# leejaeyong7/nerfacc

Hardware: AMD Instinct MI355X
Metric: rays/sec (fwd+bwd) through 128^3 occ-grid, 1M-ray batch (higher is better)
Workload: dtype f32; 1 GPU; cfg2: 1048576 image rays/GPU, 128^3 shell10 occ grid (G=1), step 2*sqrt(3)/1024, sampling+rendering fwd+bwd; rays_per_gpu=1048576, resolution=128, grid=shell10, samples_after_compaction=32244949, parallelism=ray-sharded x1, field=synthetic analytic field, native callbacks (see bench.py NativeField/TorchField)

## Files before the change

### include/nerfacc_hip.h

```cpp
#ifndef NERFACC_HIP_H
#define NERFACC_HIP_H

#include <stdint.h>

#ifdef __cplusplus
extern "C" {
#endif

#define NFA_OK 0
#define NFA_EINVAL (-1)
#define NFA_EHIP (-2)

#define NFA_MAX_GRID_LEVELS 8

typedef void *nfa_stream_t;

#define NFA_ELEM_F32 0
#define NFA_ELEM_F16 1
#define NFA_ELEM_BF16 2

const char *nfa_last_error(void);
#define NFA_VERSION 403
int nfa_version(void);
int nfa_set_tuning(const char *name, const char *value);
int nfa_device_arch(char *buf, int buflen);


int64_t nfa_cumsum_scratch_bytes(int64_t n);
int nfa_exclusive_cumsum_i64(const int64_t *cnts, int64_t n, int64_t *starts, int64_t *total,
                             void *scratch, nfa_stream_t stream);
int nfa_exclusive_cumsum_pairs_i64(const int64_t *cnts, int64_t n, int64_t *packed_info , int64_t *total,
                                   void *scratch, nfa_stream_t stream);
int nfa_exclusive_cumsum_pairs_stats_i64(const int64_t *cnts, int64_t n, int64_t *packed_info ,
                                         int64_t *total_and_stats , void *scratch, nfa_stream_t stream);

int nfa_pack_info(const int64_t *ray_indices, int64_t n, int64_t n_rays, int64_t *packed_info ,
                  int32_t *flags , void *scratch, nfa_stream_t stream);

int nfa_unpack_rows(const void *packed, const int64_t *packed_info , const uint8_t *mask, int64_t n_rays,
                    int64_t n_per_ray, int64_t n_packed, int64_t row_bytes, const void *pad_host, int32_t pad_bytes,
                    void *padded, nfa_stream_t stream);
int nfa_pack_rows(const void *padded, const int64_t *packed_info , const uint8_t *mask, int64_t n_rays,
                  int64_t n_per_ray, int64_t n_packed, int64_t row_bytes, void *packed, nfa_stream_t stream);
int nfa_mask_row_counts(const uint8_t *mask, int64_t n_rows, int64_t n_cols, int64_t *counts, nfa_stream_t stream);

int nfa_pack_bits(const uint8_t *binaries, int64_t n_cells, uint32_t *bits , nfa_stream_t stream);


int nfa_ray_aabb_intersect(const float *rays_o, const float *rays_d, int64_t n_rays,
// ... 384 lines not shown
```

### nerfacc_amd/_backend.py

```python
from __future__ import annotations

import ctypes as C
import os
import threading
from typing import Optional

import torch

from . import _build

_lock = threading.Lock()
_lib: Optional[C.CDLL] = None

_vp, _i64, _i32, _f32, _u64, _int = C.c_void_p, C.c_int64, C.c_int32, C.c_float, C.c_uint64, C.c_int


class TraverseArgs(C.Structure):
    _fields_ = [
        ("n_rays", _i64), ("rays_o", _vp), ("rays_d", _vp), ("rays_mask", _vp),
        ("n_grids", _i32), ("res", _i32 * 3), ("binaries", _vp), ("aabbs", _vp),
        ("hits", _vp), ("t_sorted", _vp), ("t_indices", _vp),
        ("near_planes", _vp), ("far_planes", _vp),
        ("step_size", _f32), ("cone_angle", _f32), ("traverse_steps_limit", _i32), ("mode", _i32),
        ("iv_vals", _vp), ("iv_ray_indices", _vp), ("iv_is_left", _vp), ("iv_is_right", _vp),
        ("iv_starts", _vp), ("iv_cnts", _vp),
        ("sm_vals", _vp), ("sm_ray_indices", _vp), ("sm_is_valid", _vp),
        ("sm_t_starts", _vp), ("sm_t_ends", _vp), ("sm_starts", _vp), ("sm_cnts", _vp),
        ("terminate_planes", _vp),
        ("ray_filter", _vp), ("ray_filter_min", _i32),
        ("bricks", _vp), ("coarse", _vp),
        ("steps_limit_dev", _vp), ("n_listed_dev", _vp), ("run_if_nonzero", _vp),
    ]


_SIGS = {
    "nfa_exclusive_cumsum_i64": [_vp, _i64, _vp, _vp, _vp, _vp],
    "nfa_exclusive_cumsum_pairs_i64": [_vp, _i64, _vp, _vp, _vp, _vp],
    "nfa_exclusive_cumsum_pairs_stats_i64": [_vp, _i64, _vp, _vp, _vp, _vp],
    "nfa_pack_info": [_vp, _i64, _i64, _vp, _vp, _vp, _vp],
    "nfa_pdf_loss_fwd": [_vp, _vp, _vp, _vp, _i64, _i32, _i32, _f32, _vp, _vp, _vp],
    "nfa_pdf_loss_bwd": [_vp, _vp, _vp, _i64, _i32, _i32, _f32, _vp, _vp, _vp, _vp],
    "nfa_pdf_loss_partials": [_i64, _i32, _i32],
    "nfa_pdf_loss_sum_fwd": [_vp, _vp, _vp, _vp, _i64, _i32, _i32, _f32, _vp, _vp, _vp],
    "nfa_pdf_loss_mean_bwd": [_vp, _vp, _vp, _i64, _i32, _i32, _f32, _vp, _vp, _vp, _vp],
    "nfa_pack_bits": [_vp, _i64, _vp, _vp],
    "nfa_unpack_rows": [_vp, _vp, _vp, _i64, _i64, _i64, _i64, _vp, _i32, _vp, _vp],
    "nfa_pack_rows": [_vp, _vp, _vp, _i64, _i64, _i64, _i64, _vp, _vp],
    "nfa_mask_row_counts": [_vp, _i64, _i64, _vp, _vp],
    "nfa_ray_aabb_intersect": [_vp, _vp, _i64, _vp, _i32, _f32, _f32, _f32, _vp, _vp, _vp, _vp],
    "nfa_ray_events": [_vp, _vp, _i64, _vp, _i32, _vp, _vp, _vp, _vp],
    "nfa_traverse_grids": [C.POINTER(TraverseArgs), _vp],
    "nfa_bricks_words": [_i32, C.POINTER(_i32)],
    "nfa_pack_bricks": [_vp, _i32, C.POINTER(_i32), _vp, _vp, _vp],
# ... 176 lines not shown
            dev = t.device
        elif t.device != dev:
            raise RuntimeError(f"nerfacc_amd: tensors on different devices ({dev} vs {t.device})")
    if dev is None:
        raise RuntimeError("nerfacc_amd: no tensor argument")
    return dev


def seg_plan(n_elems: int, n_rays: int = 0):
    t, n = _i64(0), _i64(0)
    load().nfa_seg_plan(n_elems, n_rays, C.byref(t), C.byref(n))
    return int(t.value), int(n.value)


def cumsum_scratch(n: int, device) -> torch.Tensor:
    nbytes = ((max(n, 1) + 2047) // 2048 + 1) * 8
    return torch.empty(nbytes // 8, dtype=torch.int64, device=device)
```

### nerfacc_amd/_segments.py

```python
from __future__ import annotations

import ctypes
import weakref
from dataclasses import dataclass
from typing import Optional

import torch
from torch import Tensor

from . import _backend as B


@dataclass
class SegInfo:
    packed_info: Tensor
    n_rays: int
    n_elems: int
    tiles: Optional[Tensor]
    contiguous: bool
    sorted_indices: bool = True
    n_tiles: int = 0
    trusted: bool = False


_ATTR = "_nfa_seg"
_ATTR_RI = "_nfa_seg_from_ray_indices"


def _build_tiles(packed_info: Tensor, n_elems: int, trusted: bool) -> SegInfo:
    dev = B.require_device(packed_info)
    n_rays = packed_info.shape[0]
    with torch.cuda.device(dev):
        tile_elems, n_tiles = B.seg_plan(n_elems, n_rays)
        tiles = torch.empty((int(B.load().nfa_seg_table_rows(n_tiles)), 2), dtype=torch.int64, device=dev)
        flag = None if trusted else torch.empty(1, dtype=torch.int32, device=dev)
        B.call("nfa_seg_build_tiles", B.ptr(packed_info), n_rays, n_elems, tile_elems, n_tiles, B.ptr(tiles), B.ptr(flag),
               B.stream())
        ok = True if trusted else (int(flag.item()) == 0)
    return SegInfo(packed_info, n_rays, n_elems, tiles if ok else None, ok, n_tiles=n_tiles, trusted=trusted)


def seginfo_from_packed(packed_info: Tensor, n_elems: int, trusted: bool = False) -> SegInfo:
    assert packed_info.dim() == 2 and packed_info.shape[-1] == 2, "packed_info must be 2-D with shape (B, 2)."
    cached = getattr(packed_info, _ATTR, None)
    if cached is not None and cached[0] == packed_info._version and cached[1] == n_elems:
        return cached[2]
    pi = packed_info
    if pi.dtype != torch.int64 or not pi.is_contiguous():
        pi = pi.to(torch.int64).contiguous()
    info = _build_tiles(pi, n_elems, trusted)
    try:
        setattr(packed_info, _ATTR, (packed_info._version, n_elems, info))
    except Exception:
        pass
    return info


def tag_trusted(packed_info: Tensor, n_elems: int) -> SegInfo:
    return seginfo_from_packed(packed_info, n_elems, trusted=True)


def pack_info_native(ray_indices: Tensor, n_rays: int):
    dev = B.require_device(ray_indices)
    ri = ray_indices if (ray_indices.dtype == torch.int64 and ray_indices.is_contiguous()) else \
        ray_indices.to(torch.int64).contiguous()
    with torch.cuda.device(dev):
        packed = torch.empty((n_rays, 2), dtype=torch.int64, device=dev)
        flag = torch.empty(1, dtype=torch.int32, device=dev)
        scratch = B.cumsum_scratch(n_rays, dev)
        B.call("nfa_pack_info", B.ptr(ri), ri.numel(), n_rays, B.ptr(packed), B.ptr(flag), B.ptr(scratch), B.stream())
    return packed, flag


def seginfo_from_ray_indices(ray_indices: Tensor, n_rays: int) -> SegInfo:
# ... 90 lines not shown
```

### nerfacc_amd/csrc/common.hip.h

```cpp
#pragma once
#include <hip/hip_runtime.h>
#include <stdint.h>
#include <stdio.h>
#include <stdlib.h>
#include <string.h>

#include <type_traits>

#include "../../include/nerfacc_hip.h"

#define NFA_WAVE 64

namespace nfa {

void set_error(const char *fmt, ...);

#define NFA_REQUIRE(cond, ...)                         \
    do {                                               \
        if (!(cond)) {                                 \
            nfa::set_error(__VA_ARGS__);               \
            return NFA_EINVAL;                         \
        }                                              \
    } while (0)

// ... 22 lines not shown
    int min_busy = 48;
    if (refill_env) { long c = 0; int m = 0; if (sscanf(refill_env, "%ld,%d", &c, &m) == 2 && c >= 64 && m >= 1 && m <= 64) { chunk = c / 64 * 64; min_busy = m; } }
    return RefillPlan{true, chunk, min_busy};
}

static inline hipStream_t as_stream(nfa_stream_t s) { return reinterpret_cast<hipStream_t>(s); }

__host__ __device__ static inline int64_t ceil_div64(int64_t a, int64_t b) { return (a + b - 1) / b; }

static inline unsigned grid_1d(int64_t n, int block, int64_t cap = 256 * 16)
{
    int64_t g = ceil_div64(n, block);
    if (g > cap) g = cap;
    if (g < 1) g = 1;
    return (unsigned)g;
}

static inline bool aligned16(const void *p) { return (reinterpret_cast<uintptr_t>(p) & 15) == 0; }
template <typename... P>
static inline bool all_aligned16(P... p) { return (aligned16(p) && ...); }

template <class F>
static void dispatch_bool(bool b, F &&f)
{
    if (b) f(std::true_type{});
    else f(std::false_type{});
}
template <class F>
static void dispatch_channels(int c, F &&f)
{
// ... 322 lines not shown
```

### nerfacc_amd/csrc/grid.hip

```cpp
#include <stdarg.h>

#include "common.hip.h"
#include "march.h"

namespace nfa {

static thread_local char g_err[512] = "";
void set_error(const char *fmt, ...)
{
    va_list ap;
    va_start(ap, fmt);
    vsnprintf(g_err, sizeof(g_err), fmt, ap);
    va_end(ap);
}

struct TuningKnob { char name[32]; char value[64]; };
static TuningKnob g_knobs[8];
static int g_n_knobs = 0;
const char *tuning_env(const char *name)
{
    for (int i = 0; i < g_n_knobs; ++i)
        if (strcmp(g_knobs[i].name, name) == 0) return g_knobs[i].value[0] ? g_knobs[i].value : nullptr;
    return nullptr;
}
// ... 340 lines not shown
        if (!span_cell<EMIT_RUNS, false, true, true>(a, tid, 0, 0, sp, st, ro)) return RF_WALK;
        return (a.traverse_steps_limit > 0 && st.n_samples >= a.traverse_steps_limit) ? RF_FINISH : RF_SPAN;
    }
    __device__ __forceinline__ void finish() { run_ray_close(a, ro, tid, st.t_last, st.n_samples, st.n_runs); }
};
template <bool FUSED>
__global__ __launch_bounds__(256) void traverse_refill_kernel(const nfa_traverse_args a, const RunOut ro, const int32_t chunk,
                                                              const int32_t min_busy)
{
    SpanState sp;
    BrickWalker<FUSED> w{a, ro, 0, 0, 0.0f, 0.0f, {0.0f, 0.0f, 0.0f}, {0.0f, 0.0f, 0.0f}, {0.0f, 0.0f, 0.0f}, RayState{0.0f, 0, 0, 0, -1, 0u, 0u, 0, 0}, sp};
    refill_schedule(w, ro.order, ro.order ? ro.n_order : a.n_rays, (int64_t)blockIdx.x * (blockDim.x >> 6) + (threadIdx.x >> 6), chunk, min_busy);
}

constexpr int CS_THREADS = 256;
constexpr int CS_ITEMS = 8;
constexpr int CS_BLOCK = CS_THREADS * CS_ITEMS;

__device__ __forceinline__ int64_t block_excl_scan_i64(int64_t v, int64_t &block_total, int64_t *lds )
{
    const int lane = lane_id(), wave = threadIdx.x >> 6;
    const int64_t incl = wave_incl_sum_i64(v);
    if (lane == 63) lds[wave] = incl;
    __syncthreads();
    int64_t wave_off = 0, tot = 0;
#pragma unroll
    for (int w = 0; w < CS_THREADS / 64; ++w) {
        const int64_t x = lds[w];
        if (w < wave) wave_off += x;
        tot += x;
    }
    __syncthreads();
    block_total = tot;
    return wave_off + incl - v;
}

__global__ __launch_bounds__(CS_THREADS) void cumsum_partials_kernel(const int64_t *__restrict__ in, int64_t n,
                                                                      int64_t in_stride, int64_t *__restrict__ partials)
{
    __shared__ int64_t lds[8];
    const int64_t base = (int64_t)blockIdx.x * CS_BLOCK + (int64_t)threadIdx.x * CS_ITEMS;
    int64_t s = 0;
#pragma unroll
    for (int k = 0; k < CS_ITEMS; ++k)
        if (base + k < n) s += in[(base + k) * in_stride];
    int64_t tot;
    block_excl_scan_i64(s, tot, lds);
    if (threadIdx.x == 0) partials[blockIdx.x] = tot;
}

__global__ __launch_bounds__(CS_THREADS) void cumsum_spine_kernel(int64_t *partials, int64_t n_blocks, int64_t *total)
{
    __shared__ int64_t lds[8];
    int64_t carry = 0;
    for (int64_t base = 0; base < n_blocks; base += CS_THREADS) {
        const int64_t i = base + threadIdx.x;
        const int64_t v = i < n_blocks ? partials[i] : 0;
        int64_t tot;
        const int64_t ex = block_excl_scan_i64(v, tot, lds);
        if (i < n_blocks) partials[i] = carry + ex;
        carry += tot;
    }
    if (threadIdx.x == 0 && total) *total = carry;
}

template <bool SPINE>
__global__ __launch_bounds__(CS_THREADS) void cumsum_final_kernel(const int64_t *__restrict__ in, int64_t n,
                                                                   int64_t in_stride,
                                                                   const int64_t *__restrict__ partials,
                                                                   int64_t *__restrict__ out, int pairs,
                                                                   int64_t *__restrict__ total,
                                                                   unsigned long long *__restrict__ stats = nullptr)
{
    __shared__ int64_t lds[8];
    int64_t block_off = 0;
    if (SPINE) {
        int64_t before = 0;
        for (int64_t j = threadIdx.x; j < (int64_t)blockIdx.x; j += CS_THREADS) before += partials[j];
        block_excl_scan_i64(before, block_off, lds);
    } else {
        block_off = partials[blockIdx.x];
    }
    const int64_t base = (int64_t)blockIdx.x * CS_BLOCK + (int64_t)threadIdx.x * CS_ITEMS;
    int64_t v[CS_ITEMS];
    int64_t s = 0;
#pragma unroll
    for (int k = 0; k < CS_ITEMS; ++k) {
        v[k] = (base + k < n) ? in[(base + k) * in_stride] : 0;
        s += v[k];
    }
    int64_t tot;
    int64_t run = block_off + block_excl_scan_i64(s, tot, lds);
    if (SPINE && total && blockIdx.x == gridDim.x - 1 && threadIdx.x == 0) *total = block_off + tot;
    if (SPINE && stats && (blockIdx.x & 7) == 0) {
        int64_t m = 0;
#pragma unroll
        for (int k = 0; k < CS_ITEMS; ++k) m = v[k] > m ? v[k] : m;
        for (int off = 1; off < 8; off <<= 1) { const int64_t u = __shfl_xor(m, off, 64); m = u > m ? u : m; }
        int64_t gm = (lane_id() & 7) == 0 ? m : 0;
        for (int off = 8; off < 64; off <<= 1) gm += __shfl_xor(gm, off, 64);
        if (lane_id() == 0) atomicAdd(&stats[0], (unsigned long long)gm);
        if (threadIdx.x == 0) atomicAdd(&stats[1], (unsigned long long)tot);
    }
#pragma unroll
    for (int k = 0; k < CS_ITEMS; ++k) {
        if (base + k < n) {
            if (pairs) { out[2 * (base + k)] = run; out[2 * (base + k) + 1] = v[k]; }
            else out[base + k] = run;
        }
        run += v[k];
    }
}

static int run_cumsum(const int64_t *in, int64_t n, int64_t in_stride, int64_t *out, int pairs, int64_t *total,
                      void *scratch, hipStream_t s, unsigned long long *stats = nullptr)
{
    const int64_t n_blocks = ceil_div64(n > 0 ? n : 1, CS_BLOCK);
    int64_t *partials = reinterpret_cast<int64_t *>(scratch);
    hipLaunchKernelGGL(cumsum_partials_kernel, dim3((unsigned)n_blocks), dim3(CS_THREADS), 0, s, in, n, in_stride, partials);
    if (n_blocks <= 2048) {
        hipLaunchKernelGGL(cumsum_final_kernel<true>, dim3((unsigned)n_blocks), dim3(CS_THREADS), 0, s, in, n, in_stride, partials,
                           out, pairs, total, stats);
    } else {
        hipLaunchKernelGGL(cumsum_spine_kernel, dim3(1), dim3(CS_THREADS), 0, s, partials, n_blocks, total);
        hipLaunchKernelGGL(cumsum_final_kernel<false>, dim3((unsigned)n_blocks), dim3(CS_THREADS), 0, s, in, n, in_stride, partials,
                           out, pairs, nullptr, nullptr);
    }
    NFA_CHECK_LAUNCH("exclusive_cumsum_i64");
    return NFA_OK;
}

__global__ __launch_bounds__(256) void pack_hist_kernel(const int64_t *__restrict__ ray_indices, int64_t n,
                                                        int64_t n_rays, unsigned long long *__restrict__ packed,
                                                        int32_t *__restrict__ flags)
{
    const int lane = lane_id();
    for (int64_t base = ((int64_t)blockIdx.x * blockDim.x + threadIdx.x) - lane; base < n;
         base += (int64_t)blockDim.x * gridDim.x) {
        const int64_t i = base + lane;
        const bool valid = i < n;
        const int64_t r = valid ? ray_indices[i] : -1;
        int64_t prev = __shfl_up(r, 1, NFA_WAVE);
// ... 57 lines not shown
    hipDeviceProp_t prop;
    if (hipGetDevice(&dev) != hipSuccess || hipGetDeviceProperties(&prop, dev) != hipSuccess) {
        set_error("no HIP device");
        return NFA_EHIP;
    }
    snprintf(buf, buflen, "%s", prop.gcnArchName);
    return NFA_OK;
}

int64_t nfa_cumsum_scratch_bytes(int64_t n) { return (ceil_div64(n > 0 ? n : 1, CS_BLOCK) + 1) * 8; }

int nfa_exclusive_cumsum_i64(const int64_t *cnts, int64_t n, int64_t *starts, int64_t *total, void *scratch,
                             nfa_stream_t stream)
{
    NFA_REQUIRE(n >= 0 && scratch && (n == 0 || (cnts && starts)), "exclusive_cumsum_i64: bad arguments");
    return run_cumsum(cnts, n, 1, starts, 0, total, scratch, as_stream(stream));
}

int nfa_exclusive_cumsum_pairs_i64(const int64_t *cnts, int64_t n, int64_t *packed_info, int64_t *total, void *scratch,
                                   nfa_stream_t stream)
{
    NFA_REQUIRE(n >= 0 && scratch && (n == 0 || (cnts && packed_info)), "exclusive_cumsum_pairs_i64: bad arguments");
    return run_cumsum(cnts, n, 1, packed_info, 1, total, scratch, as_stream(stream));
}

int nfa_exclusive_cumsum_pairs_stats_i64(const int64_t *cnts, int64_t n, int64_t *packed_info, int64_t *total_and_stats,
                                         void *scratch, nfa_stream_t stream)
{
    NFA_REQUIRE(n >= 0 && scratch && total_and_stats && (n == 0 || (cnts && packed_info)),
                "exclusive_cumsum_pairs_stats_i64: bad arguments");
    return run_cumsum(cnts, n, 1, packed_info, 1, total_and_stats, scratch, as_stream(stream),
                      reinterpret_cast<unsigned long long *>(total_and_stats + 1));
}

int nfa_pack_info(const int64_t *ray_indices, int64_t n, int64_t n_rays, int64_t *packed_info, int32_t *flags,
                  void *scratch, nfa_stream_t stream)
{
    NFA_REQUIRE(n >= 0 && n_rays >= 0 && flags && scratch, "pack_info: bad arguments");
    NFA_REQUIRE(n_rays == 0 || packed_info, "pack_info: packed_info is null");
    NFA_REQUIRE(n == 0 || ray_indices, "pack_info: ray_indices is null");
    hipStream_t s = as_stream(stream);
    hipLaunchKernelGGL(zero_i64_kernel, dim3(grid_1d(2 * n_rays + 1, 256)), dim3(256), 0, s, packed_info, 2 * n_rays, flags);
    if (n > 0 && n_rays > 0)
        hipLaunchKernelGGL(pack_hist_kernel, dim3(grid_1d(n, 256)), dim3(256), 0, s, ray_indices, n, n_rays,
                           reinterpret_cast<unsigned long long *>(packed_info), flags);
    NFA_CHECK_LAUNCH("pack_info");
    if (n_rays == 0) return NFA_OK;
    return run_cumsum(packed_info + 1, n_rays, 2, packed_info, 1, nullptr, scratch, s);
}

int nfa_pack_bits(const uint8_t *binaries, int64_t n_cells, uint32_t *bits, nfa_stream_t stream)
{
    NFA_REQUIRE(n_cells >= 0 && (n_cells == 0 || (binaries && bits)), "pack_bits: bad arguments");
    if (n_cells == 0) return NFA_OK;
    hipLaunchKernelGGL(pack_bits_kernel, dim3(grid_1d(n_cells, 256)), dim3(256), 0, as_stream(stream), binaries, n_cells, bits);
    NFA_CHECK_LAUNCH("pack_bits");
    return NFA_OK;
}

int nfa_ray_aabb_intersect(const float *rays_o, const float *rays_d, int64_t n_rays, const float *aabbs,
                           int32_t n_aabbs, float near_plane, float far_plane, float miss_value, float *t_mins,
                           float *t_maxs, uint8_t *hits, nfa_stream_t stream)
{
// ... 113 lines not shown
```

### nerfacc_amd/csrc/segscan.hip

```cpp
#include <stdlib.h>

#include "common.hip.h"
#include "samples.h"

namespace nfa {

constexpr int SE = 4;
constexpr int SQ = SE / 4;
constexpr int SEG_CHUNK = 64 * SE;
#ifndef NFA_SEG_TILE_ROWS
#define NFA_SEG_TILE_ROWS 256
#endif
constexpr int64_t SEG_TILE_ROWS = NFA_SEG_TILE_ROWS;
#ifndef NFA_VIS_EXP_FREE
#define NFA_VIS_EXP_FREE 1
#endif
#ifndef NFA_SEG_WAVES_PER_BLOCK
#define NFA_SEG_WAVES_PER_BLOCK 4
#endif
constexpr int SEG_WAVES_PER_BLOCK = NFA_SEG_WAVES_PER_BLOCK;

__global__ __launch_bounds__(256) void seg_build_tiles_kernel(const int64_t *__restrict__ packed_info, int64_t n_rays,
                                                              int64_t n_elems, int64_t tile_elems, int64_t n_tiles,
                                                              longlong2 *__restrict__ tiles, int32_t *__restrict__ flags)
{
    for (int64_t r = (int64_t)blockIdx.x * blockDim.x + threadIdx.x; r <= n_rays;
         r += (int64_t)blockDim.x * gridDim.x) {
        int64_t b_lo, b_hi, e_first;
        bool bad = false;
        if (r < n_rays) {
            const int64_t s = packed_info[2 * r], n = packed_info[2 * r + 1];
            int64_t s_prev = -1;
            if (r > 0) {
                const int64_t ps = packed_info[2 * r - 2], pn = packed_info[2 * r - 1];
                s_prev = ps;
                bad |= (ps + pn != s);
            }
            bad |= (n < 0) || (s < 0) || (s + n > n_elems);
            if (bad) { if (flags) atomicOr(flags, 1); continue; }
            b_lo = (s_prev < 0) ? 0 : s_prev / tile_elems + (r - 1) / SEG_TILE_ROWS + 1;
            b_hi = s / tile_elems + r / SEG_TILE_ROWS;
            e_first = s;
        } else {
            const int64_t s_prev = n_rays > 0 ? packed_info[2 * n_rays - 2] : -1;
            const int64_t n_prev = n_rays > 0 ? packed_info[2 * n_rays - 1] : 0;
            b_lo = (s_prev < 0) ? 0 : s_prev / tile_elems + (n_rays - 1) / SEG_TILE_ROWS + 1;
            b_hi = n_tiles;
            e_first = (s_prev < 0) ? 0 : s_prev + n_prev;
            if (s_prev > n_elems) { if (flags) atomicOr(flags, 1); continue; }
        }
        for (int64_t b = b_lo; b <= b_hi && b <= n_tiles; ++b) tiles[b] = make_longlong2(r, e_first);
    }
}

__host__ __device__ inline int64_t seg_table_rows(int64_t n_tiles) { return n_tiles + 1; }

struct F4 { float v[SE]; };

struct Pos {
    int64_t c;
    int32_t off;
// ... 2094 lines not shown
            op.gsig = grad_sigmas; op.grgb = grad_rgbs;
            launch_seg<-1>(op, packed_info, tiles, n_rays, n_tiles, as_stream(stream));
        });
    });
    NFA_CHECK_LAUNCH(name);
    return NFA_OK;
}

extern "C" {

void nfa_seg_plan(int64_t n_elems, int64_t n_rays, int64_t *tile_elems, int64_t *n_tiles)
{
    const int64_t t_env = tuning_env("NFA_SEG_TILE") ? atoll(tuning_env("NFA_SEG_TILE")) : 0;
    const int64_t t = t_env > 0 ? t_env : 1024;
    *tile_elems = t;
    *n_tiles = n_elems / t + (n_rays > 0 ? n_rays : 0) / SEG_TILE_ROWS + 1;
}

int64_t nfa_seg_table_rows(int64_t n_tiles) { return seg_table_rows(n_tiles); }

int nfa_seg_build_tiles(const int64_t *packed_info, int64_t n_rays, int64_t n_elems, int64_t tile_elems, int64_t n_tiles,
                        int64_t *tiles, int32_t *flags, nfa_stream_t stream)
{
    NFA_REQUIRE(n_rays >= 0 && n_elems >= 0 && tiles, "seg_build_tiles: bad arguments");
    NFA_REQUIRE(n_rays == 0 || packed_info, "seg_build_tiles: packed_info is null");
    NFA_REQUIRE(n_rays < ((int64_t)1 << 31) - 64, "seg_build_tiles: too many rays");
    NFA_REQUIRE(tile_elems >= 64 && tile_elems % 4 == 0 && n_tiles == n_elems / tile_elems + n_rays / SEG_TILE_ROWS + 1,
                "seg_build_tiles: tile_elems must be a multiple of 4 (>= 64) and n_tiles what nfa_seg_plan returns for (n_elems, n_rays)");
    hipStream_t s = as_stream(stream);
    if (flags && hipMemsetAsync(flags, 0, sizeof(int32_t), s) != hipSuccess) { set_error("seg_build_tiles: memset failed"); return NFA_EHIP; }
    hipLaunchKernelGGL(seg_build_tiles_kernel, dim3(grid_1d(n_rays + 1, 256)), dim3(256), 0, s, packed_info, n_rays,
                       n_elems, tile_elems, n_tiles, reinterpret_cast<longlong2 *>(tiles), flags);
    NFA_CHECK_LAUNCH("seg_build_tiles");
    return NFA_OK;
}

int nfa_packed_scan(int kind, int reverse, const int64_t *packed_info, const int64_t *tiles, int64_t n_tiles, int64_t n_rays,
                    int64_t n_elems, const float *inputs, float *outputs, nfa_stream_t stream)
{
    SEG_COMMON_CHECKS("packed_scan");
    NFA_REQUIRE(kind >= 0 && kind <= 3, "packed_scan: kind must be 0..3");
    if (n_elems == 0) return NFA_OK;
// ... 712 lines not shown
```

### nerfacc_amd/grid.py

```python
from __future__ import annotations

import ctypes as C
import os
from typing import Optional, Tuple

import torch
from torch import Tensor

from . import _backend as B
from ._segments import tag_const_step, tag_ray_indices, tag_trusted
from .data_specs import RayIntervals, RaySamples


@torch.no_grad()
def ray_aabb_intersect(
    rays_o: Tensor,
    rays_d: Tensor,
    aabbs: Tensor,
    near_plane: float = -float("inf"),
    far_plane: float = float("inf"),
    miss_value: float = float("inf"),
) -> Tuple[Tensor, Tensor, Tensor]:
    assert rays_o.ndim == 2 and rays_o.shape[-1] == 3
    assert rays_d.ndim == 2 and rays_d.shape[-1] == 3
    assert aabbs.ndim == 2 and aabbs.shape[-1] == 6
# ... 278 lines not shown


_SIDE_STREAMS: dict = {}


def _side_stream(dev) -> "torch.cuda.Stream":
    key = (dev.index, torch.cuda.current_stream(dev).cuda_stream)
    st = _SIDE_STREAMS.get(key)
    if st is None:
        st = _SIDE_STREAMS[key] = torch.cuda.Stream(device=dev)
    return st


SPECULATE = os.environ.get("NERFACC_AMD_SPECULATE", "1") != "0"
_SPEC_CAPACITY: dict = {}
_PINNED: dict = {}


def _pinned_meta(dev) -> Tensor:
    buf = _PINNED.get(dev.index)
    if buf is None:
        buf = _PINNED[dev.index] = torch.empty(8, dtype=torch.int64, pin_memory=True)
    return buf


CONE_RUNS = os.environ.get("NERFACC_AMD_CONE_RUNS", "1") != "0"
ALIVE_LIST_FRACTION = float(os.environ.get("NERFACC_AMD_ALIVE_FRACTION", "0.75"))
CONE_WALK = os.environ.get("NERFACC_AMD_CONE_WALK", "1") != "0"
CONE_ARENA = os.environ.get("NERFACC_AMD_CONE_ARENA", "1") != "0"
CONE_ARENA_MIN = 4096
# ... 66 lines not shown
                res3 = (C.c_int32 * 3)(*binaries.shape[1:])
                B.call("nfa_bin_rays_levels", B.ptr(rays_o), B.ptr(rays_d), n_rays, B.ptr(aabbs), binaries.shape[0], res3,
                       float(near_hint) if near_hint is not None else 0.0, B.ptr(order), B.ptr(scratch), B.ptr(meta[4:6]), B.stream())
                if not binned and not (stats_sink is not None and stats_sink.get("cells_max_over_mean", 1.0) > CONE_BIN_THRESHOLD):
                    order = None
            if CONE_WALK and _walk_supported(binaries) and min(binaries.shape[1:]) >= 4:
                arena_cap = CONE_ARENA and max(CONE_ARENA_MIN, (n_rays // 8 + 15) // 16 * 16)
                arena = torch.zeros(2 * arena_cap, dtype=torch.int64, device=dev) if arena_cap else None
                B.call("nfa_traverse_cone_walk", C.byref(a), B.ptr(_get_walk_bits(binaries)), B.ptr(run_cnts), B.ptr(runs), MAX_RUNS,
                       B.ptr(meta[3:4]), B.ptr(arena), arena_cap, B.ptr(order), 0 if order is None else order.numel(), B.stream())
            else:
                B.call("nfa_traverse_cone_runs", C.byref(a), B.ptr(run_cnts), B.ptr(runs), MAX_RUNS, B.ptr(meta[3:4]), B.ptr(order),
                       0 if order is None else order.numel(), B.stream())
        else:
            _launch(a)
        packed_info = _cumsum_packed(sm_cnts, meta[0:3], stats=True)
        cap = _SPEC_CAPACITY.get(spec_key, 0) if (SPECULATE and speculate and use_runs) else 0
        t_starts = t_ends = ray_indices = None
        if cap > 0:
            host = _pinned_meta(dev)
            main = torch.cuda.current_stream()
            ready = torch.cuda.Event(); ready.record(main)
            side = _side_stream(dev)
            with torch.cuda.stream(side):
                side.wait_event(ready)
                host[:6].copy_(meta, non_blocking=True)
                done = torch.cuda.Event(); done.record(side)
            t_starts = torch.empty(cap, dtype=torch.float32, device=dev)
            t_ends = torch.empty(cap, dtype=torch.float32, device=dev)
            ray_indices = torch.empty(cap, dtype=torch.int64, device=dev)
            B.call("nfa_expand_runs", n_rays, float(step_size), B.ptr(run_cnts), B.ptr(runs), MAX_RUNS,
                   B.ptr(packed_info), B.ptr(t_starts), B.ptr(t_ends), None, B.ptr(ray_indices), cap, B.stream())
# ... 48 lines not shown
                       MAX_RUNS, B.ptr(packed_info), B.ptr(t_starts), B.ptr(t_ends), B.ptr(ray_indices), B.stream())
                if n_arena > 0:
                    B.call("nfa_expand_cone_arena", B.ptr(arena), n_arena, float(step_size), float(cone_angle), B.ptr(packed_info),
                           B.ptr(t_starts), B.ptr(t_ends), B.ptr(ray_indices), B.stream())
            if joined is not None:
                main.wait_event(joined)
            if not (use_runs or use_cone_runs):
                a.mode = 1
                a.terminate_planes = None
                sm_starts = packed_info[:, 0].contiguous()
                a.sm_starts = B.ptr(sm_starts)
                a.sm_t_starts, a.sm_t_ends = B.ptr(t_starts), B.ptr(t_ends)
                a.sm_ray_indices = None
                _launch(a)
                B.call("nfa_fill_ray_indices", n_rays, B.ptr(packed_info), B.ptr(ray_indices), B.stream())
    info = tag_trusted(packed_info, n_sm)
    tag_ray_indices(ray_indices, n_rays, info)
    if use_runs and not masked:
        tag_const_step(t_starts, t_ends, step_size)
    out = (ray_indices, t_starts, t_ends, packed_info)
    return (*out, terminate) if return_terminate else out


def _enlarge_aabb(aabb: Tensor, factor: float) -> Tensor:
    center = (aabb[:3] + aabb[3:]) / 2
    extent = (aabb[3:] - aabb[:3]) / 2
    return torch.cat([center - extent * factor, center + extent * factor])


def _query(x: Tensor, data: Tensor, base_aabb: Tensor) -> Tuple[Tensor, Tensor]:
    lo, hi = base_aabb[:3], base_aabb[3:]
# ... 10 lines not shown
```

Measured before the change: 729.8 million rays/s.

## Fuse segment tile-table construction into the packed-info cumsum kernel

The exclusive cumsum that builds packed_info can now also write the segment tile table in the same pass, so the separate nfa_seg_build_tiles launch and its reread of packed_info are skipped on the speculative-capacity path. The cumsum kernels are also reorganised into wave-strided loads with shuffle reductions, 16-byte pair stores, and a larger single-pass spine threshold. This adds tile-boundary logic to the scan kernel and sizes the tile table from the speculative capacity, which must cover the actual sample count or the code falls back to building tiles separately.

```diff
diff --git a/include/nerfacc_hip.h b/include/nerfacc_hip.h
--- a/include/nerfacc_hip.h
+++ b/include/nerfacc_hip.h
@@ -33,6 +33,10 @@
                                    void *scratch, nfa_stream_t stream);
 int nfa_exclusive_cumsum_pairs_stats_i64(const int64_t *cnts, int64_t n, int64_t *packed_info ,
                                          int64_t *total_and_stats , void *scratch, nfa_stream_t stream);
+int nfa_exclusive_cumsum_pairs_stats_tiles_i64(const int64_t *cnts, int64_t n, int64_t *packed_info ,
+                                               int64_t *total_and_stats , void *scratch, int64_t tile_elems,
+                                               int64_t *tiles , int64_t tile_rows_cap,
+                                               nfa_stream_t stream);
 
 int nfa_pack_info(const int64_t *ray_indices, int64_t n, int64_t n_rays, int64_t *packed_info ,
                   int32_t *flags , void *scratch, nfa_stream_t stream);
diff --git a/nerfacc_amd/_backend.py b/nerfacc_amd/_backend.py
--- a/nerfacc_amd/_backend.py
+++ b/nerfacc_amd/_backend.py
@@ -37,6 +37,7 @@
     "nfa_exclusive_cumsum_i64": [_vp, _i64, _vp, _vp, _vp, _vp],
     "nfa_exclusive_cumsum_pairs_i64": [_vp, _i64, _vp, _vp, _vp, _vp],
     "nfa_exclusive_cumsum_pairs_stats_i64": [_vp, _i64, _vp, _vp, _vp, _vp],
+    "nfa_exclusive_cumsum_pairs_stats_tiles_i64": [_vp, _i64, _vp, _vp, _vp, _i64, _vp, _i64, _vp],
     "nfa_pack_info": [_vp, _i64, _i64, _vp, _vp, _vp, _vp],
     "nfa_pdf_loss_fwd": [_vp, _vp, _vp, _vp, _i64, _i32, _i32, _f32, _vp, _vp, _vp],
     "nfa_pdf_loss_bwd": [_vp, _vp, _vp, _i64, _i32, _i32, _f32, _vp, _vp, _vp, _vp],
@@ -243,5 +244,5 @@
 
 
 def cumsum_scratch(n: int, device) -> torch.Tensor:
-    nbytes = ((max(n, 1) + 2047) // 2048 + 1) * 8
-    return torch.empty(nbytes // 8, dtype=torch.int64, device=device)
+    nbytes = int(load().nfa_cumsum_scratch_bytes(n))
+    return torch.empty((nbytes + 7) // 8, dtype=torch.int64, device=device)
diff --git a/nerfacc_amd/_segments.py b/nerfacc_amd/_segments.py
--- a/nerfacc_amd/_segments.py
+++ b/nerfacc_amd/_segments.py
@@ -27,11 +27,17 @@
 _ATTR_RI = "_nfa_seg_from_ray_indices"
 
 
-def _build_tiles(packed_info: Tensor, n_elems: int, trusted: bool) -> SegInfo:
+def tile_rows_for(capacity: int, n_rays: int) -> int:
+    return B.seg_plan(max(int(capacity), 0), n_rays)[1] + 1
+
+
+def _build_tiles(packed_info: Tensor, n_elems: int, trusted: bool, prebuilt: Optional[Tensor] = None) -> SegInfo:
     dev = B.require_device(packed_info)
     n_rays = packed_info.shape[0]
     with torch.cuda.device(dev):
         tile_elems, n_tiles = B.seg_plan(n_elems, n_rays)
+        if prebuilt is not None and trusted and prebuilt.shape[0] >= n_tiles + 1:
+            return SegInfo(packed_info, n_rays, n_elems, prebuilt[:n_tiles + 1], True, n_tiles=n_tiles, trusted=True)
         tiles = torch.empty((int(B.load().nfa_seg_table_rows(n_tiles)), 2), dtype=torch.int64, device=dev)
         flag = None if trusted else torch.empty(1, dtype=torch.int32, device=dev)
         B.call("nfa_seg_build_tiles", B.ptr(packed_info), n_rays, n_elems, tile_elems, n_tiles, B.ptr(tiles), B.ptr(flag),
@@ -40,7 +46,7 @@
     return SegInfo(packed_info, n_rays, n_elems, tiles if ok else None, ok, n_tiles=n_tiles, trusted=trusted)
 
 
-def seginfo_from_packed(packed_info: Tensor, n_elems: int, trusted: bool = False) -> SegInfo:
+def seginfo_from_packed(packed_info: Tensor, n_elems: int, trusted: bool = False, tiles: Optional[Tensor] = None) -> SegInfo:
     assert packed_info.dim() == 2 and packed_info.shape[-1] == 2, "packed_info must be 2-D with shape (B, 2)."
     cached = getattr(packed_info, _ATTR, None)
     if cached is not None and cached[0] == packed_info._version and cached[1] == n_elems:
@@ -48,7 +54,7 @@
     pi = packed_info
     if pi.dtype != torch.int64 or not pi.is_contiguous():
         pi = pi.to(torch.int64).contiguous()
-    info = _build_tiles(pi, n_elems, trusted)
+    info = _build_tiles(pi, n_elems, trusted, tiles if pi is packed_info else None)
     try:
         setattr(packed_info, _ATTR, (packed_info._version, n_elems, info))
     except Exception:
@@ -56,8 +62,8 @@
     return info
 
 
-def tag_trusted(packed_info: Tensor, n_elems: int) -> SegInfo:
-    return seginfo_from_packed(packed_info, n_elems, trusted=True)
+def tag_trusted(packed_info: Tensor, n_elems: int, tiles: Optional[Tensor] = None) -> SegInfo:
+    return seginfo_from_packed(packed_info, n_elems, trusted=True, tiles=tiles)
 
 
 def pack_info_native(ray_indices: Tensor, n_rays: int):
diff --git a/nerfacc_amd/csrc/common.hip.h b/nerfacc_amd/csrc/common.hip.h
--- a/nerfacc_amd/csrc/common.hip.h
+++ b/nerfacc_amd/csrc/common.hip.h
@@ -60,6 +60,19 @@
     if (g > cap) g = cap;
     if (g < 1) g = 1;
     return (unsigned)g;
+}
+
+#ifndef NFA_SEG_TILE_ROWS
+#define NFA_SEG_TILE_ROWS 256
+#endif
+constexpr int64_t SEG_TILE_ROWS = NFA_SEG_TILE_ROWS;
+__host__ __device__ static inline int64_t seg_tile_of_ray(int64_t start, int64_t r, int64_t tile_elems, int shift = -1)
+{
+    return (shift >= 0 ? start >> shift : start / tile_elems) + r / SEG_TILE_ROWS;
+}
+__host__ __device__ static inline int64_t seg_n_tiles(int64_t n_elems, int64_t n_rays, int64_t tile_elems)
+{
+    return n_elems / tile_elems + n_rays / SEG_TILE_ROWS + 1;
 }
 
 static inline bool aligned16(const void *p) { return (reinterpret_cast<uintptr_t>(p) & 15) == 0; }
diff --git a/nerfacc_amd/csrc/grid.hip b/nerfacc_amd/csrc/grid.hip
--- a/nerfacc_amd/csrc/grid.hip
+++ b/nerfacc_amd/csrc/grid.hip
@@ -378,8 +378,27 @@
 }
 
 constexpr int CS_THREADS = 256;
-constexpr int CS_ITEMS = 8;
-constexpr int CS_BLOCK = CS_THREADS * CS_ITEMS;
+constexpr int CS_WAVES = CS_THREADS / NFA_WAVE;
+constexpr int CS_ROUNDS = 4;
+constexpr int CS_WAVE_ELEMS = NFA_WAVE * CS_ROUNDS;
+constexpr int CS_BLOCK = CS_WAVES * CS_WAVE_ELEMS;
+constexpr int64_t CS_SPINE_BLOCKS = 4096;
+constexpr int CS_PART_LOADS = 4;
+constexpr int CS_STAT_RUN = 2048;
+static_assert(CS_STAT_RUN % CS_BLOCK == 0, "a workgroup must not straddle two runs of the coherence sample");
+
+__device__ __forceinline__ int64_t wave_sum_i64(int64_t v)
+{
+#pragma unroll
+    for (int off = 32; off > 0; off >>= 1) v += __shfl_xor(v, off, NFA_WAVE);
+    return v;
+}
+__device__ __forceinline__ int64_t wave_max_i64(int64_t v)
+{
+#pragma unroll
+    for (int off = 32; off > 0; off >>= 1) { const int64_t u = __shfl_xor(v, off, NFA_WAVE); v = u > v ? u : v; }
+    return v;
+}
 
 __device__ __forceinline__ int64_t block_excl_scan_i64(int64_t v, int64_t &block_total, int64_t *lds )
 {
@@ -389,7 +408,7 @@
     __syncthreads();
     int64_t wave_off = 0, tot = 0;
 #pragma unroll
-    for (int w = 0; w < CS_THREADS / 64; ++w) {
+    for (int w = 0; w < CS_WAVES; ++w) {
         const int64_t x = lds[w];
         if (w < wave) wave_off += x;
         tot += x;
@@ -402,20 +421,29 @@
 __global__ __launch_bounds__(CS_THREADS) void cumsum_partials_kernel(const int64_t *__restrict__ in, int64_t n,
                                                                       int64_t in_stride, int64_t *__restrict__ partials)
 {
-    __shared__ int64_t lds[8];
-    const int64_t base = (int64_t)blockIdx.x * CS_BLOCK + (int64_t)threadIdx.x * CS_ITEMS;
+    __shared__ int64_t lds[CS_WAVES];
+    const int lane = lane_id(), wave = threadIdx.x >> 6;
+    const int64_t wave_base = (int64_t)blockIdx.x * CS_BLOCK + wave * CS_WAVE_ELEMS;
     int64_t s = 0;
 #pragma unroll
-    for (int k = 0; k < CS_ITEMS; ++k)
-        if (base + k < n) s += in[(base + k) * in_stride];
-    int64_t tot;
-    block_excl_scan_i64(s, tot, lds);
-    if (threadIdx.x == 0) partials[blockIdx.x] = tot;
+    for (int k = 0; k < CS_ROUNDS; ++k) {
+        const int64_t i = wave_base + k * NFA_WAVE + lane;
+        if (i < n) s += in[i * in_stride];
+    }
+    s = wave_sum_i64(s);
+    if (lane == 0) lds[wave] = s;
+    __syncthreads();
+    if (threadIdx.x == 0) {
+        int64_t tot = 0;
+#pragma unroll
+        for (int w = 0; w < CS_WAVES; ++w) tot += lds[w];
+        partials[blockIdx.x] = tot;
+    }
 }
 
 __global__ __launch_bounds__(CS_THREADS) void cumsum_spine_kernel(int64_t *partials, int64_t n_blocks, int64_t *total)
 {
-    __shared__ int64_t lds[8];
+    __shared__ int64_t lds[CS_WAVES];
     int64_t carry = 0;
     for (int64_t base = 0; base < n_blocks; base += CS_THREADS) {
         const int64_t i = base + threadIdx.x;
@@ -428,68 +456,123 @@
     if (threadIdx.x == 0 && total) *total = carry;
 }
 
-template <bool SPINE>
+struct TileOut {
+    longlong2 *tiles;
+    int64_t tile_elems;
+    int64_t rows_cap;
+    int32_t shift;
+};
+enum { CS_OUT_STARTS = 0, CS_OUT_ROWS = 1, CS_OUT_ROWS16 = 2 };
+
+template <bool SPINE, bool TILES>
 __global__ __launch_bounds__(CS_THREADS) void cumsum_final_kernel(const int64_t *__restrict__ in, int64_t n,
                                                                    int64_t in_stride,
                                                                    const int64_t *__restrict__ partials,
-                                                                   int64_t *__restrict__ out, int pairs,
+                                                                   int64_t *__restrict__ out, int out_kind,
                                                                    int64_t *__restrict__ total,
-                                                                   unsigned long long *__restrict__ stats = nullptr)
-{
-    __shared__ int64_t lds[8];
-    int64_t block_off = 0;
+                                                                   unsigned long long *__restrict__ stats, const TileOut to)
+{
+    __shared__ int64_t lds[3 * CS_WAVES];
+    const int lane = lane_id(), wave = threadIdx.x >> 6;
+    const int64_t wave_base = (int64_t)blockIdx.x * CS_BLOCK + wave * CS_WAVE_ELEMS;
+    int64_t v[CS_ROUNDS], incl[CS_ROUNDS], carry[CS_ROUNDS];
+#pragma unroll
+    for (int k = 0; k < CS_ROUNDS; ++k) {
+        const int64_t i = wave_base + k * NFA_WAVE + lane;
+        v[k] = i < n ? in[i * in_stride] : 0;
+    }
+    int64_t v_before = 0;
+    if (TILES && lane == 0 && wave_base > 0 && wave_base <= n) v_before = in[(wave_base - 1) * in_stride];
+    int64_t before = 0;
     if (SPINE) {
-        int64_t before = 0;
-        for (int64_t j = threadIdx.x; j < (int64_t)blockIdx.x; j += CS_THREADS) before += partials[j];
-        block_excl_scan_i64(before, block_off, lds);
-    } else {
-        block_off = partials[blockIdx.x];
-    }
-    const int64_t base = (int64_t)blockIdx.x * CS_BLOCK + (int64_t)threadIdx.x * CS_ITEMS;
-    int64_t v[CS_ITEMS];
-    int64_t s = 0;
-#pragma unroll
-    for (int k = 0; k < CS_ITEMS; ++k) {
-        v[k] = (base + k < n) ? in[(base + k) * in_stride] : 0;
-        s += v[k];
-    }
-    int64_t tot;
-    int64_t run = block_off + block_excl_scan_i64(s, tot, lds);
-    if (SPINE && total && blockIdx.x == gridDim.x - 1 && threadIdx.x == 0) *total = block_off + tot;
-    if (SPINE && stats && (blockIdx.x & 7) == 0) {
-        int64_t m = 0;
-#pragma unroll
-        for (int k = 0; k < CS_ITEMS; ++k) m = v[k] > m ? v[k] : m;
-        for (int off = 1; off < 8; off <<= 1) { const int64_t u = __shfl_xor(m, off, 64); m = u > m ? u : m; }
-        int64_t gm = (lane_id() & 7) == 0 ? m : 0;
-        for (int off = 8; off < 64; off <<= 1) gm += __shfl_xor(gm, off, 64);
-        if (lane_id() == 0) atomicAdd(&stats[0], (unsigned long long)gm);
-        if (threadIdx.x == 0) atomicAdd(&stats[1], (unsigned long long)tot);
-    }
-#pragma unroll
-    for (int k = 0; k < CS_ITEMS; ++k) {
-        if (base + k < n) {
-            if (pairs) { out[2 * (base + k)] = run; out[2 * (base + k) + 1] = v[k]; }
-            else out[base + k] = run;
-        }
-        run += v[k];
-    }
-}
-
-static int run_cumsum(const int64_t *in, int64_t n, int64_t in_stride, int64_t *out, int pairs, int64_t *total,
-                      void *scratch, hipStream_t s, unsigned long long *stats = nullptr)
+        for (int64_t j0 = threadIdx.x; j0 < (int64_t)blockIdx.x; j0 += CS_PART_LOADS * CS_THREADS) {
+            int64_t p[CS_PART_LOADS];
+#pragma unroll
+            for (int u = 0; u < CS_PART_LOADS; ++u) {
+                const int64_t j = j0 + u * CS_THREADS;
+                p[u] = j < (int64_t)blockIdx.x ? partials[j] : 0;
+            }
+#pragma unroll
+            for (int u = 0; u < CS_PART_LOADS; ++u) before += p[u];
+        }
+    }
+    int64_t wave_tot = 0;
+#pragma unroll
+    for (int k = 0; k < CS_ROUNDS; ++k) {
+        incl[k] = wave_incl_sum_i64(v[k]);
+        carry[k] = wave_tot;
+        wave_tot += wave_shfl(incl[k], NFA_WAVE - 1);
+    }
+    const bool sampled = SPINE && stats && ((((int64_t)blockIdx.x * CS_BLOCK / CS_STAT_RUN) & 7) == 0);
+    int64_t gm = 0;
+    if (sampled) {
+#pragma unroll
+        for (int k = 0; k < CS_ROUNDS; ++k) gm += wave_max_i64(v[k] > 0 ? v[k] : 0);
+    }
+    if (SPINE) before = wave_sum_i64(before);
+    if (lane == 0) { lds[wave] = wave_tot; lds[CS_WAVES + wave] = before; lds[2 * CS_WAVES + wave] = gm; }
+    __syncthreads();
+    int64_t off = SPINE ? 0 : partials[blockIdx.x], tot = 0, gm_sum = 0;
+#pragma unroll
+    for (int w = 0; w < CS_WAVES; ++w) {
+        const int64_t x = lds[w];
+        if (w < wave) off += x;
+        tot += x;
+        if (SPINE) off += lds[CS_WAVES + w];
+        gm_sum += lds[2 * CS_WAVES + w];
+    }
+    if (threadIdx.x == 0) {
+        if (SPINE && total && blockIdx.x == gridDim.x - 1) *total = off + tot;
+        if (sampled) { atomicAdd(&stats[0], (unsigned long long)gm_sum); atomicAdd(&stats[1], (unsigned long long)tot); }
+    }
+#pragma unroll
+    for (int k = 0; k < CS_ROUNDS; ++k) {
+        const int64_t i = wave_base + k * NFA_WAVE + lane;
+        const int64_t start = off + carry[k] + incl[k] - v[k];
+        if (i < n) {
+            if (out_kind == CS_OUT_ROWS16) store_l2(out + 2 * i, start, v[k]);
+            else if (out_kind == CS_OUT_ROWS) { out[2 * i] = start; out[2 * i + 1] = v[k]; }
+            else out[i] = start;
+        }
+        if (TILES) {
+            int64_t v_prev = wave_shfl_up(v[k], 1);
+            const int64_t v_last = k > 0 ? wave_shfl(v[k - 1], NFA_WAVE - 1) : v_before;
+            if (lane == 0) v_prev = v_last;
+            if (i < n) {
+                int64_t b = i == 0 ? 0 : seg_tile_of_ray(start - v_prev, i - 1, to.tile_elems, to.shift) + 1;
+                int64_t b_hi = seg_tile_of_ray(start, i, to.tile_elems, to.shift);
+                if (b < 0) b = 0;
+                for (; b <= b_hi && b < to.rows_cap; ++b) to.tiles[b] = make_longlong2(i, start);
+                if (i == n - 1) {
+                    const int64_t all = start + v[k];
+                    b_hi = seg_n_tiles(all >= 0 ? all : 0, n, to.tile_elems);
+                    for (; b <= b_hi && b < to.rows_cap; ++b) to.tiles[b] = make_longlong2(n, all);
+                }
+            }
+        }
+    }
+    if (TILES && n == 0 && threadIdx.x == 0)
+        for (int64_t b = 0; b <= 1 && b < to.rows_cap; ++b) to.tiles[b] = make_longlong2(0, 0);
+}
+
+static int run_cumsum(const int64_t *in, int64_t n, int64_t in_stride, int64_t *out, bool pairs, int64_t *total,
+                      void *scratch, hipStream_t s, unsigned long long *stats = nullptr, const TileOut *tiles = nullptr)
 {
     const int64_t n_blocks = ceil_div64(n > 0 ? n : 1, CS_BLOCK);
     int64_t *partials = reinterpret_cast<int64_t *>(scratch);
+    const int out_kind = !pairs ? CS_OUT_STARTS : aligned16(out) ? CS_OUT_ROWS16 : CS_OUT_ROWS;
+    const TileOut to = tiles ? *tiles : TileOut{nullptr, 1, 0, -1};
     hipLaunchKernelGGL(cumsum_partials_kernel, dim3((unsigned)n_blocks), dim3(CS_THREADS), 0, s, in, n, in_stride, partials);
-    if (n_blocks <= 2048) {
-        hipLaunchKernelGGL(cumsum_final_kernel<true>, dim3((unsigned)n_blocks), dim3(CS_THREADS), 0, s, in, n, in_stride, partials,
-                           out, pairs, total, stats);
-    } else {
-        hipLaunchKernelGGL(cumsum_spine_kernel, dim3(1), dim3(CS_THREADS), 0, s, partials, n_blocks, total);
-        hipLaunchKernelGGL(cumsum_final_kernel<false>, dim3((unsigned)n_blocks), dim3(CS_THREADS), 0, s, in, n, in_stride, partials,
-                           out, pairs, nullptr, nullptr);
-    }
+    dispatch_bool(tiles != nullptr, [&](auto T) {
+        if (n_blocks <= CS_SPINE_BLOCKS) {
+            hipLaunchKernelGGL((cumsum_final_kernel<true, decltype(T)::value>), dim3((unsigned)n_blocks), dim3(CS_THREADS), 0, s, in, n,
+                               in_stride, partials, out, out_kind, total, stats, to);
+        } else {
+            hipLaunchKernelGGL(cumsum_spine_kernel, dim3(1), dim3(CS_THREADS), 0, s, partials, n_blocks, total);
+            hipLaunchKernelGGL((cumsum_final_kernel<false, decltype(T)::value>), dim3((unsigned)n_blocks), dim3(CS_THREADS), 0, s, in, n,
+                               in_stride, partials, out, out_kind, (int64_t *)nullptr, (unsigned long long *)nullptr, to);
+        }
+    });
     NFA_CHECK_LAUNCH("exclusive_cumsum_i64");
     return NFA_OK;
 }
@@ -577,14 +660,14 @@
                              nfa_stream_t stream)
 {
     NFA_REQUIRE(n >= 0 && scratch && (n == 0 || (cnts && starts)), "exclusive_cumsum_i64: bad arguments");
-    return run_cumsum(cnts, n, 1, starts, 0, total, scratch, as_stream(stream));
+    return run_cumsum(cnts, n, 1, starts, false, total, scratch, as_stream(stream));
 }
 
 int nfa_exclusive_cumsum_pairs_i64(const int64_t *cnts, int64_t n, int64_t *packed_info, int64_t *total, void *scratch,
                                    nfa_stream_t stream)
 {
     NFA_REQUIRE(n >= 0 && scratch && (n == 0 || (cnts && packed_info)), "exclusive_cumsum_pairs_i64: bad arguments");
-    return run_cumsum(cnts, n, 1, packed_info, 1, total, scratch, as_stream(stream));
+    return run_cumsum(cnts, n, 1, packed_info, true, total, scratch, as_stream(stream));
 }
 
 int nfa_exclusive_cumsum_pairs_stats_i64(const int64_t *cnts, int64_t n, int64_t *packed_info, int64_t *total_and_stats,
@@ -592,8 +675,23 @@
 {
     NFA_REQUIRE(n >= 0 && scratch && total_and_stats && (n == 0 || (cnts && packed_info)),
                 "exclusive_cumsum_pairs_stats_i64: bad arguments");
-    return run_cumsum(cnts, n, 1, packed_info, 1, total_and_stats, scratch, as_stream(stream),
+    return run_cumsum(cnts, n, 1, packed_info, true, total_and_stats, scratch, as_stream(stream),
                       reinterpret_cast<unsigned long long *>(total_and_stats + 1));
+}
+
+int nfa_exclusive_cumsum_pairs_stats_tiles_i64(const int64_t *cnts, int64_t n, int64_t *packed_info, int64_t *total_and_stats,
+                                               void *scratch, int64_t tile_elems, int64_t *tiles, int64_t tile_rows_cap,
+                                               nfa_stream_t stream)
+{
+    NFA_REQUIRE(n >= 0 && scratch && total_and_stats && (n == 0 || (cnts && packed_info)),
+                "exclusive_cumsum_pairs_stats_tiles_i64: bad arguments");
+    NFA_REQUIRE(tile_rows_cap >= 0 && (tile_rows_cap == 0 || tiles), "exclusive_cumsum_pairs_stats_tiles_i64: bad tile table");
+    NFA_REQUIRE(n < ((int64_t)1 << 31) - 64, "exclusive_cumsum_pairs_stats_tiles_i64: too many rays");
+    NFA_REQUIRE(tile_elems >= 64 && tile_elems % 4 == 0, "exclusive_cumsum_pairs_stats_tiles_i64: tile_elems must be a multiple of 4 (>= 64)");
+    const bool pow2 = (tile_elems & (tile_elems - 1)) == 0;
+    const TileOut to{reinterpret_cast<longlong2 *>(tiles), tile_elems, tile_rows_cap, pow2 ? __builtin_ctzll((unsigned long long)tile_elems) : -1};
+    return run_cumsum(cnts, n, 1, packed_info, true, total_and_stats, scratch, as_stream(stream),
+                      reinterpret_cast<unsigned long long *>(total_and_stats + 1), &to);
 }
 
 int nfa_pack_info(const int64_t *ray_indices, int64_t n, int64_t n_rays, int64_t *packed_info, int32_t *flags,
@@ -609,7 +707,7 @@
                            reinterpret_cast<unsigned long long *>(packed_info), flags);
     NFA_CHECK_LAUNCH("pack_info");
     if (n_rays == 0) return NFA_OK;
-    return run_cumsum(packed_info + 1, n_rays, 2, packed_info, 1, nullptr, scratch, s);
+    return run_cumsum(packed_info + 1, n_rays, 2, packed_info, true, nullptr, scratch, s);
 }
 
 int nfa_pack_bits(const uint8_t *binaries, int64_t n_cells, uint32_t *bits, nfa_stream_t stream)
diff --git a/nerfacc_amd/csrc/segscan.hip b/nerfacc_amd/csrc/segscan.hip
--- a/nerfacc_amd/csrc/segscan.hip
+++ b/nerfacc_amd/csrc/segscan.hip
@@ -8,10 +8,6 @@
 constexpr int SE = 4;
 constexpr int SQ = SE / 4;
 constexpr int SEG_CHUNK = 64 * SE;
-#ifndef NFA_SEG_TILE_ROWS
-#define NFA_SEG_TILE_ROWS 256
-#endif
-constexpr int64_t SEG_TILE_ROWS = NFA_SEG_TILE_ROWS;
 #ifndef NFA_VIS_EXP_FREE
 #define NFA_VIS_EXP_FREE 1
 #endif
@@ -38,13 +34,13 @@
             }
             bad |= (n < 0) || (s < 0) || (s + n > n_elems);
             if (bad) { if (flags) atomicOr(flags, 1); continue; }
-            b_lo = (s_prev < 0) ? 0 : s_prev / tile_elems + (r - 1) / SEG_TILE_ROWS + 1;
-            b_hi = s / tile_elems + r / SEG_TILE_ROWS;
+            b_lo = (s_prev < 0) ? 0 : seg_tile_of_ray(s_prev, r - 1, tile_elems) + 1;
+            b_hi = seg_tile_of_ray(s, r, tile_elems);
             e_first = s;
         } else {
             const int64_t s_prev = n_rays > 0 ? packed_info[2 * n_rays - 2] : -1;
             const int64_t n_prev = n_rays > 0 ? packed_info[2 * n_rays - 1] : 0;
-            b_lo = (s_prev < 0) ? 0 : s_prev / tile_elems + (n_rays - 1) / SEG_TILE_ROWS + 1;
+            b_lo = (s_prev < 0) ? 0 : seg_tile_of_ray(s_prev, n_rays - 1, tile_elems) + 1;
             b_hi = n_tiles;
             e_first = (s_prev < 0) ? 0 : s_prev + n_prev;
             if (s_prev > n_elems) { if (flags) atomicOr(flags, 1); continue; }
@@ -2169,7 +2165,7 @@
     const int64_t t_env = tuning_env("NFA_SEG_TILE") ? atoll(tuning_env("NFA_SEG_TILE")) : 0;
     const int64_t t = t_env > 0 ? t_env : 1024;
     *tile_elems = t;
-    *n_tiles = n_elems / t + (n_rays > 0 ? n_rays : 0) / SEG_TILE_ROWS + 1;
+    *n_tiles = seg_n_tiles(n_elems, n_rays > 0 ? n_rays : 0, t);
 }
 
 int64_t nfa_seg_table_rows(int64_t n_tiles) { return seg_table_rows(n_tiles); }
@@ -2180,7 +2176,7 @@
     NFA_REQUIRE(n_rays >= 0 && n_elems >= 0 && tiles, "seg_build_tiles: bad arguments");
     NFA_REQUIRE(n_rays == 0 || packed_info, "seg_build_tiles: packed_info is null");
     NFA_REQUIRE(n_rays < ((int64_t)1 << 31) - 64, "seg_build_tiles: too many rays");
-    NFA_REQUIRE(tile_elems >= 64 && tile_elems % 4 == 0 && n_tiles == n_elems / tile_elems + n_rays / SEG_TILE_ROWS + 1,
+    NFA_REQUIRE(tile_elems >= 64 && tile_elems % 4 == 0 && n_tiles == seg_n_tiles(n_elems, n_rays, tile_elems),
                 "seg_build_tiles: tile_elems must be a multiple of 4 (>= 64) and n_tiles what nfa_seg_plan returns for (n_elems, n_rays)");
     hipStream_t s = as_stream(stream);
     if (flags && hipMemsetAsync(flags, 0, sizeof(int32_t), s) != hipSuccess) { set_error("seg_build_tiles: memset failed"); return NFA_EHIP; }
diff --git a/nerfacc_amd/grid.py b/nerfacc_amd/grid.py
--- a/nerfacc_amd/grid.py
+++ b/nerfacc_amd/grid.py
@@ -8,7 +8,7 @@
 from torch import Tensor
 
 from . import _backend as B
-from ._segments import tag_const_step, tag_ray_indices, tag_trusted
+from ._segments import tag_const_step, tag_ray_indices, tag_trusted, tile_rows_for
 from .data_specs import RayIntervals, RaySamples
 
 
@@ -317,6 +317,7 @@
 
 SPECULATE = os.environ.get("NERFACC_AMD_SPECULATE", "1") != "0"
 _SPEC_CAPACITY: dict = {}
+FUSE_TILE_TABLE = os.environ.get("NERFACC_AMD_FUSE_TILE_TABLE", "1") != "0"
 _PINNED: dict = {}
 
 
@@ -413,8 +414,18 @@
                        0 if order is None else order.numel(), B.stream())
         else:
             _launch(a)
-        packed_info = _cumsum_packed(sm_cnts, meta[0:3], stats=True)
         cap = _SPEC_CAPACITY.get(spec_key, 0) if (SPECULATE and speculate and use_runs) else 0
+        tiles = None
+        if cap > 0 and FUSE_TILE_TABLE:
+            tile_elems = B.seg_plan(0, n_rays)[0]
+            tiles = torch.empty((tile_rows_for(cap, n_rays), 2), dtype=torch.int64, device=dev)
+            packed_info = torch.empty((n_rays, 2), dtype=torch.int64, device=dev)
+            scratch = B.cumsum_scratch(n_rays, dev)
+            B.call_group("nfa_exclusive_cumsum_pairs_stats_i64", lambda: B.call(
+                "nfa_exclusive_cumsum_pairs_stats_tiles_i64", B.ptr(sm_cnts), n_rays, B.ptr(packed_info), B.ptr(meta[0:3]),
+                B.ptr(scratch), tile_elems, B.ptr(tiles), tiles.shape[0], B.stream()))
+        else:
+            packed_info = _cumsum_packed(sm_cnts, meta[0:3], stats=True)
         t_starts = t_ends = ray_indices = None
         if cap > 0:
             host = _pinned_meta(dev)
@@ -493,7 +504,7 @@
                 a.sm_ray_indices = None
                 _launch(a)
                 B.call("nfa_fill_ray_indices", n_rays, B.ptr(packed_info), B.ptr(ray_indices), B.stream())
-    info = tag_trusted(packed_info, n_sm)
+    info = tag_trusted(packed_info, n_sm, tiles)
     tag_ray_indices(ray_indices, n_rays, info)
     if use_runs and not masked:
         tag_const_step(t_starts, t_ends, step_size)
```

After: 717.7 million rays/s. -1.7%, worse.
